# EryiXie/PlaneRecNet

Measured on AMD Instinct MI355X. Metric: img/s fwd+bwd @480×640 ResNet101-DCN, 1/2/4/8 MI355X + roofline %, higher is better.
Workload: dtype f32 (tensors and accumulation fp32; plain GEMMs and the tap-walked 4x4/s2, 1x1/s2 and sub-pixel convolutions >= 300 tiles: 2xfp16-piece split MFMA, fp32 accumulate; fp32-only rate in fp32_only_run)

## Files before the change

include/prn.h:

```cpp
#ifndef PRN_H
#define PRN_H
#include <stdint.h>
#ifdef __cplusplus
extern "C" {
#endif

#define PRN_BN_SPLITS 32

int prn_version(void);
const char* prn_last_error(void);

enum { PRN_IN_ZERO = 0, PRN_IN_REFLECT = 1, PRN_IN_UP2_REFLECT = 2, PRN_IN_DILATED = 3, PRN_IN_UP2_PHASE = 4,
       PRN_IN_EMBED1 = 5  };
enum { PRN_EPI_NONE = 0, PRN_EPI_RELU = 1, PRN_EPI_SIGMOID = 2 };

enum { PRN_SPLIT_OFF = 0, PRN_SPLIT_PLAN = 1, PRN_SPLIT_ALWAYS = 2 };
enum { PRN_PIECES_BF16 = 0, PRN_PIECES_F16 = 16 };
typedef struct prn_gemm_opts {
  int32_t split_mode;
  int32_t split_kind;
  int32_t split_products;
  int32_t split_min_tiles;
  float split_min_gflop;
  int32_t wgrad_wgs;
// ... 4 lines not shown

typedef struct prn_conv_desc {
  int32_t B, C, H, W;
  int32_t M;
  int32_t KH, KW;
  int32_t stride, pad;
  int32_t Ho, Wo;
  int32_t in_mode;
  int32_t dil;
  int32_t epilogue;
  int32_t ystride;
  int32_t yH, yW;
  int32_t reserved;
  prn_gemm_opts opts;
} prn_conv_desc;

int64_t prn_conv2d_fwd_ws_bytes(const prn_conv_desc* d);
int prn_conv2d_kernel_kind(const prn_conv_desc* d);
int prn_conv2d_fwd_partials(const prn_conv_desc* d, int64_t* offset_bytes);
int prn_gemm_pipe(int M, int K, int B, int HW, int nz, const prn_gemm_opts* opts);
int64_t prn_split_images_bytes(int M, int K, int nz);
int prn_split_prepare(const float* w, void* images, int M, int K, int nz, int kind, void* stream);
int prn_split_prepare_batched(const void* items_dev, int n_items, int64_t total_blocks, int64_t total_row_blocks, int kind, void* stream);
int prn_conv2d_fwd(const prn_conv_desc* d, const float* x, const float* w, const float* bias,
                   const float* addend, float* y, void* ws, void* stream);
#define PRN_TILE_COUNTERS 4096
int prn_conv2d_fwd_counted(const prn_conv_desc* d, const float* x, const float* w, const void* w_images, const float* bias, const float* addend, float* y,
                           void* ws, unsigned* counters, void* stream, int phase);
#define PRN_MAX_SEGMENTS 6
typedef struct prn_ragged {
  int32_t nseg;
  int32_t H[PRN_MAX_SEGMENTS], W[PRN_MAX_SEGMENTS];
} prn_ragged;
int prn_conv2d_fwd_ragged(const prn_conv_desc* d, const prn_ragged* rg, const float* x, const float* w, const float* bias,
                          const float* addend, float* y, void* stream);
int64_t prn_conv2d_wgrad_ragged_ws_bytes(const prn_conv_desc* d, const prn_ragged* rg);
int prn_conv2d_wgrad_ragged(const prn_conv_desc* d, const prn_ragged* rg, const float* x, const float* dy, float* dw, void* ws,
                            void* stream);

int prn_conv2d_fwd_phase(const prn_conv_desc* d, const float* x, const float* w, const float* bias,
                         const float* addend, float* y, void* ws, void* stream, int phase);

int prn_weight_flip_transpose(const float* w, float* wt, int M, int C, int KH, int KW, void* stream);

typedef struct prn_flip_item {
  const float* src;
// ... 274 lines not shown
```

planerecnet_amd/_lib.py:

```python
import ctypes
import os

_HERE = os.path.dirname(os.path.abspath(__file__))
LIB_PATH = os.environ.get("PRN_LIB") or os.path.join(_HERE, "libprn_hip.so")

c_int, c_float, c_void_p, c_i64 = ctypes.c_int, ctypes.c_float, ctypes.c_void_p, ctypes.c_int64


class GemmOpts(ctypes.Structure):
    _fields_ = [("split_mode", ctypes.c_int32), ("split_kind", ctypes.c_int32), ("split_products", ctypes.c_int32), ("split_min_tiles", ctypes.c_int32),
                ("split_min_gflop", ctypes.c_float), ("wgrad_wgs", ctypes.c_int32), ("wgrad_target", ctypes.c_int32), ("wgrad_split", ctypes.c_int32)]

    def key(self):
        return (self.split_mode, self.split_kind, self.split_products, self.split_min_tiles, self.split_min_gflop, self.wgrad_wgs, self.wgrad_target, self.wgrad_split)


SPLIT_OFF, SPLIT_PLAN, SPLIT_ALWAYS = 0, 1, 2
PIECES_BF16, PIECES_F16 = 0, 16


class ConvDesc(ctypes.Structure):
    _fields_ = [(n, ctypes.c_int32) for n in
                ("B", "C", "H", "W", "M", "KH", "KW", "stride", "pad", "Ho", "Wo", "in_mode", "dil", "epilogue", "ystride", "yH", "yW", "reserved")] + [
                    ("opts", GemmOpts)]
# ... 18 lines not shown
    _fields_ = [(n, ctypes.c_void_p) for n in (
        "w1", "w2", "w3", "wd", "b2", "w1_img", "w3_img", "wd_img", "u2", "u2_img", "w1_t", "w2_t", "w3_t", "wd_t", "w1_t_img", "w3_t_img", "wd_t_img", "ut2", "ut2_img",
        "w27", "b27", "w27_t", "w2_cols_t", "w2_cols_t_img")] + [(n, ctypes.c_void_p * 4) for n in ("gamma", "beta", "running_mean", "running_var")]


IN_ZERO, IN_REFLECT, IN_UP2_REFLECT, IN_DILATED, IN_UP2_PHASE, IN_EMBED1 = 0, 1, 2, 3, 4, 5
EPI_NONE, EPI_RELU, EPI_SIGMOID = 0, 1, 2
BN_SPLITS = 32

P = c_void_p
_DP = ctypes.POINTER(ConvDesc)
_OP = ctypes.POINTER(GemmOpts)
SIGNATURES = {
    "prn_version": (c_int, []),
    "prn_last_error": (ctypes.c_char_p, []),
    "prn_conv2d_fwd_ws_bytes": (c_i64, [_DP]),
    "prn_conv2d_kernel_kind": (c_int, [_DP]),
    "prn_conv2d_fwd_partials": (c_int, [_DP, ctypes.POINTER(c_i64)]),
    "prn_gemm_opts_default": (None, [_OP]),
    "prn_gemm_pipe": (c_int, [c_int, c_int, c_int, c_int, c_int, _OP]),
    "prn_split_images_bytes": (c_i64, [c_int, c_int, c_int]),
    "prn_split_prepare": (c_int, [P, P, c_int, c_int, c_int, c_int, P]),
    "prn_split_prepare_batched": (c_int, [P, c_int, c_i64, c_i64, c_int, P]),
    "prn_conv2d_fwd": (c_int, [_DP, P, P, P, P, P, P, P]),
    "prn_conv2d_fwd_ragged": (c_int, [_DP, P, P, P, P, P, P, P]),
    "prn_conv2d_wgrad_ragged_ws_bytes": (c_i64, [_DP, P]),
    "prn_conv2d_wgrad_ragged": (c_int, [_DP, P, P, P, P, P, P]),
    "prn_gn_relu_fwd_ragged": (c_int, [P, P, P, P, P, c_int, c_int, c_int, P, c_int, c_float, P]),
    "prn_gn_relu_bwd_ragged": (c_int, [P, P, P, P, P, P, P, P, c_int, c_int, c_int, P, c_int, P]),
    "prn_conv2d_fwd_phase": (c_int, [_DP, P, P, P, P, P, P, P, c_int]),
    "prn_conv2d_fwd_counted": (c_int, [_DP, P, P, P, P, P, P, P, P, P, c_int]),
    "prn_conv2d_wgrad_phase": (c_int, [_DP, P, P, P, P, P, c_int]),
    "prn_weight_flip_transpose": (c_int, [P, P, c_int, c_int, c_int, c_int, P]),
    "prn_weight_flip_transpose_batched": (c_int, [P, c_int, c_i64, P]),
    "prn_winograd_tiles": (c_i64, [c_int, c_int, c_int]),
    "prn_winograd_weights_batched": (c_int, [P, c_int, c_i64, P]),
    "prn_winograd_input": (c_int, [P, P, c_int, c_int, c_int, c_int, c_int, P]),
    "prn_gemm_batched_ws_bytes": (c_i64, [c_int, c_int, c_int, c_int, _OP]),
    "prn_gemm_batched": (c_int, [c_int, c_int, c_int, c_int, P, P, P, P, P, _OP, P]),
    "prn_winograd_output": (c_int, [P, P, P, P, c_int, c_int, c_int, c_int, c_int, P]),
    "prn_winograd_output_bn_fwd": (c_int, [P] * 8 + [c_int] * 4 + [c_float, c_float, c_int, P]),
    "prn_winograd_output_bn_bwd": (c_int, [P] * 8 + [c_int] * 5 + [P]),
    "prn_winograd_wgrad_ws_bytes": (c_i64, [c_int] * 5 + [_OP]),
    "prn_winograd_dy": (c_int, [P, P, c_int, c_int, c_int, c_int, P]),
    "prn_gemm_batched_nt_splits": (c_int, [c_int] * 4 + [_OP]),
    "prn_gemm_batched_nt_kind": (c_int, [c_int] * 4 + [_OP]),
# ... 131 lines not shown
```

planerecnet_amd/blocks.py:

```python
import ctypes
import os
import sys

import torch

from . import _lib, ops, profiling
from ._lib import lib, check

ENABLED = os.environ.get("PRN_BLOCKS", "1") == "1"
HANDOVER = os.environ.get("PRN_BLOCK_HANDOVER", "1") == "1"
SCATTER_ACCUMULATE = os.environ.get("PRN_SCATTER_ACC", "1") == "1"
STATS = {"fwd": 0, "bwd": 0, "resolved": 0, "vouched": 0, "scatter_acc": 0}

BLK_WINOGRAD, BLK_HANDOVER, BLK_KEEP_V, BLK_SCATTER_ACC = 1, 2, 4, 8
CONV2_DIRECT, CONV2_WINOGRAD, CONV2_DCN = 0, 1, 2
(I_SAVE, I_GSAVE, I_FWD_WS, I_BWD_WS, I_HO, I_WO, I_CONV2, I_KEEPS_V, I_A1, I_V, I_A2, I_OM, I_TABLE, I_D1, I_D2, I_D3, I_DD, I_DOM, I_BN_FLOATS, I_HANDOVERS,
 I_W1_IMG, I_W3_IMG, I_WD_IMG, I_W1T_IMG, I_W3T_IMG, I_WDT_IMG, I_U_IMG, I_COLT_IMG, INFO_COUNT) = range(29)

_SCRATCH = {}
_F32 = torch.float32
_empty = torch.empty


def scratch(nbytes, dev):
# ... 199 lines not shown
        save = _empty(st.save_n, device=dev, dtype=_F32)
        ws = scratch(st.fwd_ws, dev)
        rc = lib.prn_bottleneck_train_fwd(st.plan_ref, st.params_ref, x.data_ptr(), y.data_ptr(), save.data_ptr(), ws.data_ptr(), ops._raw_stream(dev.index))
        if rc:
            check(rc, "prn_bottleneck_train_fwd")
        torch._C._increment_version(st.stat_bufs)
        for m in st.bns:
            ops._count_batch(m)
        ctx.save_for_backward(x, y, save)
        ctx.st, ctx.keep, ctx.vs = st, st.keep, vs
        STATS["fwd"] += 1
        if hand_back:
            ctx.set_materialize_grads(False)
            return y, x0
        return y

    @staticmethod
    def backward(ctx, dy, dfork=None):
        x, y, save = ctx.saved_tensors
        st = ctx.st
        ps = st.ps
        if dy is None:
            return (dfork,) + (None,) * (3 + len(ps))
        if [w._version for w in st.convw] != ctx.vs:
            raise RuntimeError("a parameter of a Bottleneck block was modified between its forward and its backward pass")
        dev = x.device
        if not dy.is_contiguous():
            dy = dy.contiguous()
        info = st.info
        acc = 0
        if dfork is not None and st.hb and SCATTER_ACCUMULATE and dfork.is_contiguous() and dfork._base is None and dfork.shape == x.shape \
                and dfork.dtype == _F32 and dfork._use_count() <= _OWNED[0] and sys.getrefcount(dfork) <= _OWNED[1]:
            dx, acc, dfork = dfork, 1, None
            STATS["scatter_acc"] += 1
        else:
            dx = torch.empty_like(x)
        gsave = _empty(st.gsave_n, device=dev, dtype=_F32)
        bn_buf = _empty(st.bn_n, device=dev, dtype=_F32)
        ws = scratch(st.bwd_ws, dev)
        rc = lib.prn_bottleneck_train_bwd(st.plan_ref, st.params_ref, x.data_ptr(), y.data_ptr(), dy.data_ptr(), dx.data_ptr(), acc, save.data_ptr(), gsave.data_ptr(),
                                          bn_buf.data_ptr(), ws.data_ptr(), ops._raw_stream(dev.index))
        if rc:
            check(rc, "prn_bottleneck_train_bwd")
        ctx.keep = None
        STATS["bwd"] += 1
        if dfork is not None:
# ... 121 lines not shown
```

planerecnet_amd/csrc/prn_gemm_split.hip:

```cpp
#include "prn_common.h"
#include <stdlib.h>

namespace {

typedef __attribute__((ext_vector_type(8))) __bf16 bf16x8_t;
typedef __attribute__((ext_vector_type(16))) float f32x16_t;
typedef int i32x4_t __attribute__((ext_vector_type(4)));
typedef float f32x4_t __attribute__((ext_vector_type(4)));

constexpr int BM = 128, BK = 32;
constexpr int IMG_U4 = 1536;

__device__ __forceinline__ void split2(float x0, float x1, unsigned& h, unsigned& m, unsigned& l) {
  const unsigned u0 = __float_as_uint(x0), u1 = __float_as_uint(x1);
  const float r0 = x0 - __uint_as_float(u0 & 0xffff0000u), r1 = x1 - __uint_as_float(u1 & 0xffff0000u);
  const unsigned v0 = __float_as_uint(r0), v1 = __float_as_uint(r1);
  const float s0 = r0 - __uint_as_float(v0 & 0xffff0000u), s1 = r1 - __uint_as_float(v1 & 0xffff0000u);
  h = __builtin_amdgcn_perm(u1, u0, 0x07060302u);
  m = __builtin_amdgcn_perm(v1, v0, 0x07060302u);
  l = __builtin_amdgcn_perm(__float_as_uint(s1), __float_as_uint(s0), 0x07060302u);
}

__global__ void split_prepare_kernel(const float* __restrict__ w, uint4* __restrict__ img, int M, int K, long long zw, int mtiles, int kslices, long long total) {
  const long long i = (long long)blockIdx.x * 256 + threadIdx.x;
// ... 510 lines not shown
  const long long i = ((long long)blockIdx.x - it.first) * 256 + threadIdx.x;
  if (i >= total) return;
  const int* ex = (const int*)((const char*)it.dst + (long long)it.nz * mtiles * kslices * IMG16_U4 * 16);
  const int g = i % 4; const int r = (i / 4) % 128; const long long t = i / 512;
  const int ks = t % kslices; const long long zm = t / kslices; const int mt = zm % mtiles; const long long z = zm / mtiles;
  const int m = mt * 128 + r, k0 = ks * 32 + g * 8;
  const int sh = 14 - ex[z * (mtiles * 128) + m];
  float v[8];
  const float* wr = it.src + z * (long long)it.M * it.K + (long long)m * it.K + k0;
  if (m < it.M && k0 + 8 <= it.K && (it.K & 3) == 0 && (reinterpret_cast<uintptr_t>(it.src) & 15) == 0) {
    const float4 a = *reinterpret_cast<const float4*>(wr), b = *reinterpret_cast<const float4*>(wr + 4);
    v[0] = ldexpf(a.x, sh); v[1] = ldexpf(a.y, sh); v[2] = ldexpf(a.z, sh); v[3] = ldexpf(a.w, sh);
    v[4] = ldexpf(b.x, sh); v[5] = ldexpf(b.y, sh); v[6] = ldexpf(b.z, sh); v[7] = ldexpf(b.w, sh);
  } else {
#pragma unroll
    for (int j = 0; j < 8; ++j) v[j] = (m < it.M && k0 + j < it.K) ? ldexpf(wr[j], sh) : 0.f;
  }
  uint4 h, l;
  split2_f16(v[0], v[1], h.x, l.x); split2_f16(v[2], v[3], h.y, l.y); split2_f16(v[4], v[5], h.z, l.z); split2_f16(v[6], v[7], h.w, l.w);
  uint4* o = it.dst + t * IMG16_U4;
  o[g * 128 + r] = h; o[(4 + g) * 128 + r] = l;
}

}

int prn_split_gemm_plan(int M, int K, int B, int HW, int nz, const prn_gemm_opts* o) {
  if (o == nullptr || o->split_mode == PRN_SPLIT_OFF) return 0;
  if (M <= 0 || K <= 0 || B <= 0 || HW <= 0 || nz <= 0) return 0;
  if ((int64_t)K * HW >= (1LL << 29) || (int64_t)M * HW >= (1LL << 29)) return 0;
  const int mtiles = cdiv(M, 128), kslices = cdiv(K, 32);
  const int64_t tiles = (int64_t)mtiles * cdiv(HW, 128) * B * nz;
  int splits = 1;
  if (tiles < 300) {
    splits = (int)(640 / (tiles > 0 ? tiles : 1));
    if (splits > kslices / 8) splits = kslices / 8;
    static const int smax = prn_env_int("PRN_SPLIT_KSPLIT_MAX", 3);
    const int wide = splits > 4 ? 4 : splits;
    if (splits > smax) splits = smax;
    if (o->split_mode == PRN_SPLIT_PLAN && tiles * splits < o->split_min_tiles && tiles * wide >= o->split_min_tiles) splits = wide;
    if (splits < 1) splits = 1;
  }
  if (o->split_mode == PRN_SPLIT_ALWAYS) return splits;
  if ((int64_t)mtiles * 128 * 4 > (int64_t)M * 5) return 0;
  if (2.0 * M * K * (double)HW * B * nz < (double)o->split_min_gflop * 1e9) return 0;
  if (tiles * splits < o->split_min_tiles) return 0;
  return splits;
}
extern "C" void prn_gemm_opts_default(prn_gemm_opts* o) {
  if (!o) return;
  o->split_mode = PRN_SPLIT_PLAN; o->split_kind = PRN_PIECES_F16; o->split_products = 3; o->split_min_tiles = 300; o->split_min_gflop = 4.0f;
  o->wgrad_wgs = 0; o->wgrad_target = 0; o->wgrad_split = PRN_SPLIT_PLAN;
}
extern "C" int64_t prn_split_images_bytes(int M, int K, int nz) {
  if (M <= 0 || K <= 0 || nz <= 0) return -1;
  return prn_split_gemm_image_bytes(M, K, nz);
}
extern "C" int prn_split_prepare_batched(const void* items_dev, int n_items, int64_t total_blocks, int64_t total_row_blocks, int kind, void* stream) {
  PRN_REQUIRE(items_dev && n_items > 0 && total_blocks > 0 && total_blocks < (1LL << 31), "prn_split_prepare_batched: bad arguments");
  PRN_REQUIRE(kind == PRN_PIECES_F16 || kind == PRN_PIECES_BF16, "prn_split_prepare_batched: kind is PRN_PIECES_F16 or PRN_PIECES_BF16");
  if (kind == PRN_PIECES_F16) {
    PRN_REQUIRE(total_row_blocks > 0 && total_row_blocks < (1LL << 31), "prn_split_prepare_batched: the fp16 piece format needs the row-block count");
    hipLaunchKernelGGL(split16_rowmax_batched_kernel, dim3((unsigned)total_row_blocks), dim3(256), 0, (hipStream_t)stream, (const PrepItem*)items_dev, n_items);
    hipLaunchKernelGGL(split16_prepare_batched_kernel, dim3((unsigned)total_blocks), dim3(256), 0, (hipStream_t)stream, (const PrepItem*)items_dev, n_items);
    PRN_CHECK_LAUNCH("prn_split_prepare_batched/f16");
    return 0;
  }
  hipLaunchKernelGGL(split_prepare_batched_kernel, dim3((unsigned)total_blocks), dim3(256), 0, (hipStream_t)stream, (const PrepItem*)items_dev, n_items);
  PRN_CHECK_LAUNCH("prn_split_prepare_batched");
  return 0;
}
namespace {
int cut_weight(const float* w, void* images, int M, int K, int nz, long long zw, int kind, hipStream_t st, const char* who, int taps = 1) {
  const int mtiles = cdiv(M, 128), kslices = cdiv(K, 32);
  const long long ptotal = (long long)nz * mtiles * kslices * 512;
  if (kind == PRN_PIECES_F16) {
    int* ex = (int*)((char*)images + (int64_t)nz * mtiles * kslices * IMG16_U4 * 16);
    const long long rows = (long long)nz * mtiles * 128;
    hipLaunchKernelGGL(split16_rowmax_kernel, dim3(cdiv(rows, 4)), dim3(256), 0, st, w, ex, M, K, zw, mtiles * 128, rows);
    hipLaunchKernelGGL(split16_prepare_kernel, dim3(cdiv(ptotal, 256)), dim3(256), 0, st, w, (uint4*)images, (const int*)ex, M, K, zw, mtiles, kslices, ptotal, taps);
  } else {
    hipLaunchKernelGGL(split_prepare_kernel, dim3(cdiv(ptotal, 256)), dim3(256), 0, st, w, (uint4*)images, M, K, zw, mtiles, kslices, ptotal);
  }
  PRN_CHECK_LAUNCH(who);
  return 0;
}
}
extern "C" int prn_split_prepare(const float* w, void* images, int M, int K, int nz, int kind, void* stream) {
  PRN_REQUIRE(w && images && M > 0 && K > 0 && nz > 0 && (reinterpret_cast<uintptr_t>(images) & 15) == 0, "prn_split_prepare: bad arguments");
  PRN_REQUIRE(kind == PRN_PIECES_F16 || kind == PRN_PIECES_BF16, "prn_split_prepare: kind is PRN_PIECES_F16 or PRN_PIECES_BF16");
  return cut_weight(w, images, M, K, nz, (long long)M * K, kind, (hipStream_t)stream, "prn_split_prepare");
}
// ... 106 lines not shown
```

planerecnet_amd/ops.py:

```python
import ctypes

import os
import threading
import weakref

import torch

from . import _lib, profiling
from ._lib import ConvDesc, GemmOpts, IN_ZERO, IN_REFLECT, IN_UP2_REFLECT, IN_DILATED, IN_UP2_PHASE, IN_EMBED1, EPI_NONE, EPI_RELU, EPI_SIGMOID, lib, check


_SIDE = {}
WGRAD_ASYNC = bool(int(os.environ.get("PRN_WGRAD_ASYNC", "0")))


WGRAD_WGS_ASYNC = os.environ.get("PRN_WGRAD_WGS_ASYNC", "512")


_POLICY = {"split_mode": int(os.environ.get("PRN_SPLIT_GEMM", "1")),
           "kind": _lib.PIECES_BF16 if os.environ.get("PRN_SPLIT_KIND", "f16") == "bf16" else _lib.PIECES_F16,
           "products": int(os.environ.get("PRN_SPLIT16_PRODUCTS", "3")),
           "min_gflop": float(os.environ.get("PRN_SPLIT_MIN_GFLOP", "4.0")),
           "min_tiles": int(os.environ.get("PRN_SPLIT_MIN_TILES", os.environ.get("PRN_SPLIT_MIN_TILES_EVAL", "300"))),
           "wgrad_wgs": int(os.environ.get("PRN_WGRAD_WGS", "0") or 0),
# ... 517 lines not shown
            SPLIT_STATS["hits"] += 1
            return _p(e.images)
        if cur is None or e.dims != (M, K, nz, kind):
            _split_drop(ptr, stamp=False)
            e = None
    if e is None:
        owner = t if isinstance(t, torch.nn.Parameter) else (t._base if isinstance(t._base, torch.nn.Parameter) else None)
        if owner is None and _stamp_of(ptr) is None:
            SPLIT_STATS["uncached"] += 1
            return None
        if owner is not None and owner.data_ptr() != ptr:
            return None
        e = _SplitEntry()
        e.owner = weakref.ref(owner) if owner is not None else None
        e.tensor = None if owner is not None else t
        e.ptr, e.dims = ptr, (M, K, nz, kind)
        nb = lib.prn_split_images_bytes(M, K, nz)
        e.images = torch.empty(nb, device=t.device, dtype=torch.uint8)
        _SPLIT_IMG[ptr] = e
        _SPLIT_ITEMS[0] = None
        OPERAND_EPOCH[0] += 1
        if owner is not None:
            weakref.finalize(owner, lambda p=ptr, r=e: _split_drop(p) if _SPLIT_IMG.get(p) is r else None)
    check(lib.prn_split_prepare(ctypes.c_void_p(ptr), _p(e.images), M, K, nz, kind, _stream()), "prn_split_prepare")
    e.stamp = _split_state(e)
    SPLIT_STATS["cuts"] += 1
    if os.environ.get("PRN_SPLIT_DEBUG"):
        SPLIT_STATS.setdefault("who", {}).setdefault((M, K, nz, "param" if e.owner is not None else "derived"), []).append(SPLIT_STATS["refreshes"])
    return _p(e.images)


def split_images_ptr(t, M, K, nz, cols=None):
    r = split_images(t, M, K, nz, cols)
    return None if r is None else r.value


def split_refresh_all():
    if SPLIT_CACHE == "eval" or SPLIT_CACHE in ("0", False):
        return
    if _SPLIT_POLICY.get("mode", "eval") != "train":
        return
    dead = [p for p, e in _SPLIT_IMG.items() if _split_state(e) is None]
    for p in dead:
        _split_drop(p)
    if not _SPLIT_IMG:
        return
    kind = _POLICY["kind"]
    for e in [e for e in _SPLIT_IMG.values() if e.dims[3] != kind]:
        _split_drop(e.ptr, stamp=False)
    entries = list(_SPLIT_IMG.values())
    if not entries:
        return
    if _SPLIT_ITEMS[0] is None or _SPLIT_ITEMS[1] != [id(e) for e in entries]:
        items, blocks, rblocks = _prep_items(entries, entries[0].images.device)
        _SPLIT_ITEMS[0], _SPLIT_ITEMS[1], _SPLIT_ITEMS[2] = items, [id(e) for e in entries], (blocks, rblocks)
    check(lib.prn_split_prepare_batched(_p(_SPLIT_ITEMS[0]), len(entries), _SPLIT_ITEMS[2][0], _SPLIT_ITEMS[2][1], kind, _stream()), "prn_split_prepare_batched")
    for e in entries:
        e.stamp = _split_state(e)
    SPLIT_STATS["refreshes"] += 1


def conv_fwd_raw(x, w2d, bias, addend, M, K, stride, pad, Ho, Wo, mode=IN_ZERO, dil=1, epi=EPI_NONE, scatter2=None):
    B, C, H, W = x.shape
    if scatter2 is None:
        y = torch.empty(B, M, Ho, Wo, device=x.device, dtype=torch.float32)
        d_, ref, nbytes, _, _ = _desc(B, C, H, W, M, K, stride, pad, Ho, Wo, mode, dil, epi)
        wimg = split_images(w2d, M, C, 1, (B, Ho * Wo)) if (d_.kind >= 2 and K == 1 and stride == 1) else None
    else:
        wimg = None
        y = torch.zeros(B, M, scatter2[0], scatter2[1], device=x.device, dtype=torch.float32)
        _, ref, nbytes, _, _ = _desc(B, C, H, W, M, K, stride, pad, Ho, Wo, mode, dil, epi, 2, scatter2[0], scatter2[1])
    ws = torch.empty(nbytes // 4, device=x.device, dtype=torch.float32) if nbytes else None
    cnt = _counters(x.device) if (nbytes and FUSED_SPLIT_SUM) else None
    if profiling._enabled:
        kind = lib.prn_conv2d_kernel_kind(ref)
        direct = kind == 1
        split = kind >= 2
        nb_ = 4.0 * (x.numel() + w2d.numel() + y.numel() + (addend.numel() if addend is not None else 0))
        fl = 2.0 * M * C * K * K * B * Ho * Wo / (dil * dil)
        with profiling.span("conv3x3_direct" if direct else ("split_gemm_kernel" if split else "conv_igemm_kernel"), "hbm" if direct else "mfma",
                            nb_ if direct else (split_products() * fl if split else fl), ref=None if direct else fl, nbytes=nb_,
                            tag=None if direct else ("conv", C, H, W, M, K, stride, mode, dil, B)):
# ... 38 lines not shown

def conv_wgrad_grouped_raw(xs, dys, M, K, stride, pad, mode):
    G = len(xs)
    B, C, H, W = xs[0].shape
    Ho, Wo = dys[0].shape[2:]
    dev = xs[0].device
    _, ref, _, _, _ = _desc(B, C, H, W, M, K, stride, pad, Ho, Wo, mode)
    nbytes = lib.prn_conv2d_wgrad_grouped_ws_bytes(ref, G)
    if nbytes < 0:
        raise RuntimeError(lib.prn_last_error().decode())
    dw = torch.empty(G, M, C, K, K, device=dev, dtype=torch.float32)
    ws = _wspace(nbytes, dev)
    px = (ctypes.c_void_p * G)(*[t.data_ptr() for t in xs])
    pdy = (ctypes.c_void_p * G)(*[t.data_ptr() for t in dys])
    check(lib.prn_conv2d_wgrad_grouped(ref, G, px, pdy, _p(dw), _p(ws), _stream()), "prn_conv2d_wgrad_grouped")
    return dw


_FLIP_USED = set()


def flip_transpose(w):
    _FLIP_USED.add(w.data_ptr())
    e = _FLIPPED.get(w.data_ptr())
    if e is not None and tuple(t._version for t in e[0]) == e[1] and e[2].shape[1] == w.shape[0]:
        return e[2]
    M, C, KH, KW = w.shape
    wt = torch.empty(C, M, KH, KW, device=w.device, dtype=torch.float32)
    check(lib.prn_weight_flip_transpose(_p(w), _p(wt), M, C, KH, KW, _stream()), "prn_weight_flip_transpose")
    return wt


_FLIPPED = {}


class FlippedWeights:

    def __init__(self, weights):
        self.weights = [(e[0], tuple(int(v) for v in e[1])) for e in weights]
        self.data = [e[2] if len(e) > 2 else e[0] for e in weights]
        self.guards = [(e[0],) + tuple(e[3] if len(e) > 3 else ()) for e in weights]
        self.ptrs = None

    def _build(self):
        import numpy as np
        dev = self.weights[0][0].device
        total = sum(M * C * KH * KW for _, (M, C, KH, KW) in self.weights)
        self.flat = torch.empty(total, device=dev, dtype=torch.float32)
        items = np.zeros(len(self.weights), dtype=np.dtype([("src", "u8"), ("dst", "u8"), ("M", "i4"), ("C", "i4"), ("KH", "i4"), ("KW", "i4"),
                                                             ("first", "i8")]))
        self.views, first, blocks = [], 0, 0
        for i, ((_, (M, C, KH, KW)), w) in enumerate(zip(self.weights, self.data)):
            assert w.is_contiguous() and w.numel() == M * C * KH * KW and w.dtype == torch.float32
            v = self.flat[first:first + w.numel()].view(C, M, KH, KW)
            items[i] = (w.data_ptr(), v.data_ptr(), M, C, KH, KW, blocks)
            self.views.append(v)
            first += w.numel()
            blocks += ((M + 31) // 32) * ((C + 31) // 32)
        self.items = torch.from_numpy(items.view(np.uint8).reshape(-1).copy()).to(dev)
        self.total = blocks
        self.ptrs = [w.data_ptr() for w in self.data]
        OPERAND_EPOCH[0] += 1
        for k in [k for k, o in BATCHED.items() if o == id(self)]:
            del BATCHED[k]
        for v in self.views:
            BATCHED[v.data_ptr()] = id(self)

    def refresh(self):
        if not self.weights:
            return
        if self.ptrs is None or any(w.data_ptr() != p for w, p in zip(self.data, self.ptrs)):
            for p in (self.ptrs or []):
                _FLIPPED.pop(p, None)
            for v in (getattr(self, "views", None) or []):
                _split_drop(v.data_ptr())
            self._build()
        check(lib.prn_weight_flip_transpose_batched(_p(self.items), len(self.weights), self.total, _stream()), "prn_weight_flip_transpose_batched")
        for gd, d, v in zip(self.guards, self.data, self.views):
            _FLIPPED[d.data_ptr()] = (gd, tuple(t._version for t in gd), v)
            _stamp(v)


WINOGRAD = bool(int(os.environ.get("PRN_WINOGRAD", "1")))
WINOGRAD_WGRAD = bool(int(os.environ.get("PRN_WINOGRAD_WGRAD", "1")))
WINOGRAD_MIN_TILES = int(os.environ.get("PRN_WINOGRAD_MIN_TILES", "128"))
_WINO = {}


def winograd_ok(B, C, H, W, M, K, stride, pad, mode, epi):
    return (WINOGRAD and K == 3 and stride == 1 and pad == 1 and mode in (IN_ZERO, IN_REFLECT) and epi in (EPI_NONE, EPI_RELU)
            and W % 4 == 0 and H >= 8 and C >= 64 and M >= 64 and B * ((H + 3) // 4) * (W // 4) >= WINOGRAD_MIN_TILES)


def _winograd_items(entries, dev):
    import numpy as np
    items = np.zeros(len(entries), dtype=np.dtype([("src", "u8"), ("u", "u8"), ("ut", "u8"), ("M", "i4"), ("C", "i4"), ("first", "i8")]))
    blocks = 0
    for i, (w, M, C, U, Ut) in enumerate(entries):
        items[i] = (w.data_ptr(), U.data_ptr() if U is not None else 0, Ut.data_ptr() if Ut is not None else 0, M, C, blocks)
# ... 45 lines not shown


class WinogradWeights:

    def __init__(self, weights):
        self.weights = [w for w in weights]
        self.ptrs = None

    def _build(self):
        dev = self.weights[0].device
        total = sum(w.numel() * 4 for w in self.weights)
        self.flat_u = torch.empty(total, device=dev, dtype=torch.float32)
        self.flat_ut = torch.empty(total, device=dev, dtype=torch.float32)
        self.views, entries, first = [], [], 0
        for w in self.weights:
            M, C = w.shape[:2]
            assert w.is_contiguous() and tuple(w.shape[2:]) == (3, 3) and w.dtype == torch.float32
            n = 36 * M * C
            U, Ut = self.flat_u[first:first + n].view(36, M, C), self.flat_ut[first:first + n].view(36, C, M)
            self.views.append((U, Ut))
            entries.append((w, M, C, U, Ut))
            first += n
        self.items, self.total = _winograd_items(entries, dev)
        self.ptrs = [w.data_ptr() for w in self.weights]
        OPERAND_EPOCH[0] += 1
        for k in [k for k, o in BATCHED.items() if o == id(self)]:
            del BATCHED[k]
        for U, Ut in self.views:
            BATCHED[U.data_ptr()] = BATCHED[Ut.data_ptr()] = id(self)

    def refresh(self):
        if not self.weights or not WINOGRAD:
            return
        if self.ptrs is None or any(w.data_ptr() != p for w, p in zip(self.weights, self.ptrs)):
            for p in (self.ptrs or []):
                _wino_pop(p)
            self._build()
        check(lib.prn_winograd_weights_batched(_p(self.items), len(self.weights), self.total, _stream()), "prn_winograd_weights_batched")
        for w, (U, Ut) in zip(self.weights, self.views):
            _wino_store(w, U, Ut)


_WINO_WG_WS = {}
WINOGRAD_SPLIT_MIN_TILES = int(os.environ.get("PRN_SPLIT_WINO_MIN_TILES", "0"))
SPLIT_SKIP = set(filter(None, os.environ.get("PRN_SPLIT_SKIP", "").split(",")))
WINOGRAD_KEEP_V = int(os.environ.get("PRN_WINOGRAD_KEEP_V", str(128 << 20)))


def conv3x3_winograd_raw(x, U, bias, addend, M, mode=IN_ZERO, epi=EPI_NONE, keep=None):
    B, C, H, W = x.shape
    if mode == IN_EMBED1:
        H, W = H + 2, W + 4
    P = lib.prn_winograd_tiles(B, H, W)
    y = torch.empty(B, M, H, W, device=x.device, dtype=torch.float32)
    split_ok = "wino" not in SPLIT_SKIP and gemm_pipe(M, C, 1, P, 36) >= 1 and ((M + 127) // 128) * ((P + 127) // 128) * 36 >= WINOGRAD_SPLIT_MIN_TILES
    uimg = split_images(U, M, C, 36, (1, P)) if split_ok else None
    oref = opts_ref() if split_ok else None
    wkey = ("wino-fwd", B, C, H, W, M, opts_key() if split_ok else None)
    nb_ws = _WINO_WG_WS.get(wkey)
    if nb_ws is None:
        nb_ws = _WINO_WG_WS[wkey] = lib.prn_conv3x3_winograd_ws_bytes(B, C, H, W, M, oref)
        if nb_ws < 0:
            raise RuntimeError(lib.prn_last_error().decode())
# ... 35 lines not shown
            check(lib.prn_conv3x3_winograd_wgrad(*args, 1), "prn_conv3x3_winograd_wgrad")
        w16 = lib.prn_gemm_batched_nt_kind(M, C, P, 36, oref) == 2
        with profiling.span("wgrad16_kernel" if w16 else "conv_wgrad_kernel", "mfma", (split_products() if w16 else 1.0) * 2.0 * 36 * M * C * P, 2.0 * 9 * M * C * B * H * W,
                            tag=("wino-wgrad-products", C, H, W, M, 3, 1, mode, 1, B)):
            check(lib.prn_conv3x3_winograd_wgrad(*args, 2), "prn_conv3x3_winograd_wgrad")
        with profiling.span("winograd_dw_kernel", "hbm", float(nbytes) - 4.0 * 36 * (C + M) * P + 4.0 * dw.numel(), 0.0):
            check(lib.prn_conv3x3_winograd_wgrad(*args, 3), "prn_conv3x3_winograd_wgrad")
    else:
        check(lib.prn_conv3x3_winograd_wgrad(*args, 0), "prn_conv3x3_winograd_wgrad")
    return dw


def channel_sum(g):
    B, C, H, W = g.shape
    out = torch.empty(C, device=g.device, dtype=torch.float32)
    ws = _wspace(8 * C * _lib.BN_SPLITS, g.device, torch.float64)
    check(lib.prn_channel_sum(_p(g), _p(out), _p(ws), B, C, H * W, _stream()), "prn_channel_sum")
    return out


def conv_dgrad_raw(dy, w, x_shape, stride, pad, mode, addend=None):
    B, C, H, W = x_shape
    M, _, K, _ = w.shape
    if mode == IN_ZERO and winograd_ok(B, M, H, W, C, K, stride, pad, IN_ZERO, EPI_NONE) and tuple(dy.shape[2:]) == (H, W):
        return conv3x3_winograd_raw(dy, winograd_weights(w)[1], None, addend, C)
    wt = flip_transpose(w)
    if mode == IN_REFLECT and W % 4 == 0 and tuple(dy.shape[2:]) == (H, W) and winograd_ok(B, M, H + 2, W + 4, C, K, 1, 1, IN_ZERO, EPI_NONE):
        dp = conv3x3_winograd_raw(dy, winograd_weights(w)[1], None, None, C, IN_EMBED1)
        dx = torch.empty(B, C, H, W, device=dy.device, dtype=torch.float32)
        check(lib.prn_pad_fold_pitched(_p(dp), _p(dx), B, C, H, W, W + 4, _stream()), "prn_pad_fold_pitched")
        return dx if addend is None else dx + addend
    if mode in (IN_REFLECT, IN_UP2_REFLECT):
        Hv, Wv = (2 * H, 2 * W) if mode == IN_UP2_REFLECT else (H, W)
        dp = conv_fwd_raw(dy, wt, None, None, C, K, 1, 2, Hv + 2, Wv + 2)
        dx = torch.empty(B, C, H, W, device=dy.device, dtype=torch.float32)
        check(lib.prn_pad_fold(_p(dp), _p(dx), B, C, H, W, 1 if mode == IN_UP2_REFLECT else 0, _stream()), "prn_pad_fold")
        return dx if addend is None else dx + addend
    if stride == 1:
        return conv_fwd_raw(dy, wt, None, addend, C, K, 1, K - 1 - pad, H, W)
    if stride != 2:
        raise RuntimeError("conv dgrad: stride %d not implemented" % stride)
    if K == 1 and pad == 0 and addend is None:
        return conv_fwd_raw(dy, wt, None, None, C, 1, 1, 0, dy.shape[2], dy.shape[3], scatter2=(H, W))
    if K == 1 and pad == 0:
        return conv_fwd_raw(dy, wt, None, None, C, 1, 1, 0, dy.shape[2], dy.shape[3], scatter2=(H, W)) + addend
    return conv_fwd_raw(dy, wt, None, addend, C, K, 1, K - 1 - pad, H, W, IN_DILATED, 2)
# ... 684 lines not shown
class _RaggedConv(torch.autograd.Function):
    @staticmethod
    def forward(ctx, xp, w, bias, rs):
        _dev(xp, w, bias)
        xp, w, bias = _c(xp), _c(w), _c(bias)
        M, C, K, _ = w.shape
        assert xp.numel() == rs.pixels * C, (xp.shape, w.shape, rs.sizes)
        P = rs.winograd(C, M, K)
        y = _ragged_winograd_raw(xp, winograd_weights(w)[0], bias, None, rs, C, M, P) if P else _ragged_conv_raw(xp, w, bias, None, rs, C, M, K)
        ctx.save_for_backward(xp, w)
        ctx.rs, ctx.has_bias = rs, bias is not None
        ctx.bias = bias
        return y

    @staticmethod
    def backward(ctx, dy):
        xp, w = ctx.saved_tensors
        rs = ctx.rs
        dy = _c(dy)
        M, C, K, _ = w.shape
        dx = dw = db = None
        P = rs.winograd(C, M, K)
        if ctx.needs_input_grad[0]:
            dx = _ragged_winograd_raw(dy, winograd_weights(w)[1], None, None, rs, M, C, P) if P else _ragged_conv_raw(dy, flip_transpose(w), None, None, rs, M, C, K)
        def wgrad():
            if P and WINOGRAD_WGRAD:
                oref = opts_ref()
                key = (rs.key, C, M, opts_key())
                nb = _WINO_WG_WS.get(key)
                if nb is None:
                    nb = _WINO_WG_WS[key] = lib.prn_winograd_wgrad_ragged_ws_bytes(rs.ref, rs.B, C, M, oref)
                ws = torch.empty(nb // 4, device=xp.device, dtype=torch.float32)
                dwo = torch.empty_like(w)
                with profiling.span("conv3x3_winograd_wgrad_ragged", "mfma", 2.0 * 36 * M * C * P, 2.0 * 9 * M * C * rs.pixels):
                    check(lib.prn_conv3x3_winograd_wgrad_ragged(_p(xp), _p(dy), _p(dwo), _p(ws), rs.ref, rs.B, C, M, oref, _stream()), "prn_conv3x3_winograd_wgrad_ragged")
                return dwo
            _, ref, nbytes = _rdesc(rs, C, M, K)
            ws = torch.empty(max(nbytes // 4, 1), device=xp.device, dtype=torch.float32)
            dwo = torch.empty_like(w)
            with profiling.span("conv_wgrad_kernel", "mfma", 2.0 * M * C * K * K * rs.pixels):
                check(lib.prn_conv2d_wgrad_ragged(ref, rs.ref, _p(xp), _p(dy), _p(dwo), _p(ws), _stream()), "prn_conv2d_wgrad_ragged")
            return dwo
        if _defer(ctx.needs_input_grad[1], w):
            _deferred_wgrad(w, (xp, dy), wgrad)
        elif ctx.needs_input_grad[1]:
            dw = wgrad()
# ... 129 lines not shown
```

planerecnet_amd/planerecnet.py:

```python
import os

import torch
import torch.nn as nn
import torch.nn.functional as F

from . import ops, timer
from .backbone import can_fold, construct_backbone, conv_bn, folded_bn
from .config import cfg
from .fpn import FPN
from .funcs import bias_init_with_prob
from .nms import mask_nms, matrix_nms


_COORD = {}


def _coord_channels(feat):
    B, _, h, w = feat.shape
    key = (B, h, w, feat.device)
    c = _COORD.get(key)
    if c is None:
        xr = torch.linspace(-1, 1, w, device=feat.device)
        yr = torch.linspace(-1, 1, h, device=feat.device)
        y, x = torch.meshgrid(yr, xr, indexing="ij")
# ... 51 lines not shown
            dcns = [m for m in self.modules() if isinstance(m, DeformableConv2d)]
            dcn_w = {id(m.regular_conv.weight) for m in dcns}
            dcn_om = {id(c.weight) for m in dcns for c in (m.offset_conv, m.modulator_conv)}
            items = []
            for m in self.modules():
                if isinstance(m, nn.Conv2d) and m.weight.requires_grad and m.weight.is_cuda and id(m.weight) not in dcn_om:
                    M, C, KH, KW = m.weight.shape
                    items.append((m.weight, (M, C * KH * KW, 1, 1) if id(m.weight) in dcn_w else (M, C, KH, KW)))
            for m in dcns:
                if m.offset_conv.weight.requires_grad and m.offset_conv.weight.is_cuda:
                    w27 = m._merged()[0]
                    items.append((m.offset_conv.weight, tuple(w27.shape), w27, (m.modulator_conv.weight,)))
            self.__dict__["_flip_dcn"] = [(m, e[2]) for m, e in zip([m for m in dcns if m.offset_conv.weight.requires_grad and m.offset_conv.weight.is_cuda],
                                                                     [e for e in items if len(e) > 2])]
            fw = self.__dict__["_flipped"] = ops.FlippedWeights(items)
            self.__dict__["_flip_steps"] = 0
        self.__dict__["_flip_steps"] += 1
        if self.__dict__["_flip_steps"] == 3:
            used = [(w, shp, d, gd[1:]) for (w, shp), d, gd in zip(fw.weights, fw.data, fw.guards) if d.data_ptr() in ops._FLIP_USED]
            if used and len(used) < len(fw.weights):
                for d in fw.data:
                    ops._FLIPPED.pop(d.data_ptr(), None)
                fw = self.__dict__["_flipped"] = ops.FlippedWeights(used)
        fw.refresh()
        mine = self.__dict__.get("_param_ids")
        if mine is None:
            mine = self.__dict__["_param_ids"] = {id(p) for p in self.parameters()}
        seen = [w for w in ops.winograd_seen() if id(w) in mine]
        ww = self.__dict__.get("_wino")
        if seen and (ww is None or len(ww.weights) != len(seen)):
            ww = self.__dict__["_wino"] = ops.WinogradWeights(seen)
        if ww is not None:
            ww.refresh()
        ops.split_refresh_all()
        ops.vouch_refreshed([t for gd in fw.guards for t in gd])
        if ww is not None:
            ops.vouch_refreshed(ww.weights)

    def forward(self, x):
        if x.is_cuda:
            ops.split_gemm_policy("train" if self.training else "eval")
        if self.training and torch.is_grad_enabled() and x.is_cuda:
            self._refresh_dgrad_weights()
        with timer.env("backbone"):
            enc = self.backbone(x)
        with timer.env("fpn"):
            feats, fenc = self.fpn([enc[i] for i in self.fpn_indices], return_inputs=True)
            enc = list(enc)
            for i, f in zip(self.fpn_indices, fenc):
                enc[i] = f
        with timer.env("instance head"):
            ins_feats, feats[0] = self.split_feats([feats[f] for f in range(len(self.instance_in_features))], fork=True)
            cate_pred, kernel_pred = self.inst_head(ins_feats)
        with timer.env("mask head"):
            mask_pred = self.mask_head([feats[f] for f in range(len(self.mask_in_features))])
        with timer.env("depth_decoder"):
            depth_pred = self.depth_decoder([enc[i] for i in self.depth_decoder_indices], mask_pred, kernel_pred)
        with timer.env("Inferencing"):
            if self.training:
                return mask_pred, cate_pred, kernel_pred, depth_pred
            from .metrics import category_scores
            return self.inference(mask_pred, category_scores(cate_pred), kernel_pred, depth_pred, x)

    @staticmethod
    def split_feats(feats, fork=False):
        h, w = feats[0].shape[2:]
        if fork:
            r, f0 = ops.resize_bilinear_fork(feats[0], (int(h * 0.5), int(w * 0.5)))
            return (r, feats[1], feats[2], feats[3]), f0
        return (ops.resize_bilinear(feats[0], (int(h * 0.5), int(w * 0.5))), feats[1], feats[2], feats[3])

    def _flush_bn_counters(self):
        for m in self.modules():
            if isinstance(m, nn.BatchNorm2d):
                ops.flush_batch_count(m)

    def state_dict(self, *args, **kwargs):
        self._flush_bn_counters()
        return super().state_dict(*args, **kwargs)

    def load_state_dict(self, *args, **kwargs):
        for m in self.modules():
# ... 349 lines not shown
```

Measured before the change: 194.6.

## Refresh backward-only derived weights on a side stream and fuse split-image prep

```diff
diff --git a/include/prn.h b/include/prn.h
--- a/include/prn.h
+++ b/include/prn.h
@@ -50,6 +50,13 @@
 int64_t prn_split_images_bytes(int M, int K, int nz);
 int prn_split_prepare(const float* w, void* images, int M, int K, int nz, int kind, void* stream);
 int prn_split_prepare_batched(const void* items_dev, int n_items, int64_t total_blocks, int64_t total_row_blocks, int kind, void* stream);
+typedef struct prn_refresh_item {
+  const float* src;
+  void* images;
+  int32_t M, K, nz, pad;
+  int64_t first;
+} prn_refresh_item;
+int prn_weight_refresh_batched(const prn_refresh_item* items_host, const void* items_dev, int n_items, int kind, void* stream);
 int prn_conv2d_fwd(const prn_conv_desc* d, const float* x, const float* w, const float* bias,
                    const float* addend, float* y, void* ws, void* stream);
 #define PRN_TILE_COUNTERS 4096
diff --git a/planerecnet_amd/_lib.py b/planerecnet_amd/_lib.py
--- a/planerecnet_amd/_lib.py
+++ b/planerecnet_amd/_lib.py
@@ -64,6 +64,7 @@
     "prn_split_images_bytes": (c_i64, [c_int, c_int, c_int]),
     "prn_split_prepare": (c_int, [P, P, c_int, c_int, c_int, c_int, P]),
     "prn_split_prepare_batched": (c_int, [P, c_int, c_i64, c_i64, c_int, P]),
+    "prn_weight_refresh_batched": (c_int, [P, P, c_int, c_int, P]),
     "prn_conv2d_fwd": (c_int, [_DP, P, P, P, P, P, P, P]),
     "prn_conv2d_fwd_ragged": (c_int, [_DP, P, P, P, P, P, P, P]),
     "prn_conv2d_wgrad_ragged_ws_bytes": (c_i64, [_DP, P]),
diff --git a/planerecnet_amd/blocks.py b/planerecnet_amd/blocks.py
--- a/planerecnet_amd/blocks.py
+++ b/planerecnet_amd/blocks.py
@@ -245,6 +245,7 @@
         ps = st.ps
         if dy is None:
             return (dfork,) + (None,) * (3 + len(ps))
+        ops.backward_join()
         if [w._version for w in st.convw] != ctx.vs:
             raise RuntimeError("a parameter of a Bottleneck block was modified between its forward and its backward pass")
         dev = x.device
diff --git a/planerecnet_amd/csrc/prn_gemm_split.hip b/planerecnet_amd/csrc/prn_gemm_split.hip
--- a/planerecnet_amd/csrc/prn_gemm_split.hip
+++ b/planerecnet_amd/csrc/prn_gemm_split.hip
@@ -556,6 +556,87 @@
   o[g * 128 + r] = h; o[(4 + g) * 128 + r] = l;
 }
 
+constexpr int RF_HELD = 4;
+__device__ __forceinline__ void refresh_load8(const float* wr, bool vec, bool row_ok, int k0, int K, float* v) {
+  if (row_ok && vec && k0 + 8 <= K) {
+    const float4 a = *reinterpret_cast<const float4*>(wr + k0), b = *reinterpret_cast<const float4*>(wr + k0 + 4);
+    v[0] = a.x; v[1] = a.y; v[2] = a.z; v[3] = a.w; v[4] = b.x; v[5] = b.y; v[6] = b.z; v[7] = b.w;
+  } else {
+#pragma unroll
+    for (int j = 0; j < 8; ++j) v[j] = (row_ok && k0 + j < K) ? wr[k0 + j] : 0.f;
+  }
+}
+template <int KIND>
+__global__ __launch_bounds__(256) void weight_refresh_kernel(const prn_refresh_item* __restrict__ items, int n) {
+  __shared__ float rowmx[4][16];
+  int lo = 0, hi = n - 1;
+  const long long blk = blockIdx.x;
+  while (lo < hi) { const int mid = (lo + hi + 1) >> 1; if (items[mid].first <= blk) lo = mid; else hi = mid - 1; }
+  const prn_refresh_item it = items[lo];
+  const int mtiles = (it.M + 127) / 128, kslices = (it.K + 31) / 32, Mpad = mtiles * 128;
+  const long long u = blk - it.first;
+  const int rg = (int)(u % 8); const long long zm = u / 8; const int mt = (int)(zm % mtiles); const long long z = zm / mtiles;
+  if (z >= it.nz) return;
+  const int lane = threadIdx.x & 63, wave = threadIdx.x >> 6;
+  const int g = lane & 3, r = rg * 16 + (lane >> 2), m = mt * 128 + r;
+  const bool row_ok = m < it.M;
+  const bool vec = (it.K & 3) == 0 && (reinterpret_cast<uintptr_t>(it.src) & 15) == 0;
+  const float* wr = it.src + z * (long long)it.M * it.K + (long long)(row_ok ? m : 0) * it.K;
+  float held[RF_HELD][8];
+#pragma unroll
+  for (int i = 0; i < RF_HELD; ++i) {
+    const int ks = wave + 4 * i;
+    refresh_load8(wr, vec, row_ok && ks < kslices, ks * 32 + g * 8, it.K, held[i]);
+  }
+  int sh = 0;
+  if (KIND == PRN_PIECES_F16) {
+    float mx = 0.f;
+#pragma unroll
+    for (int i = 0; i < RF_HELD; ++i)
+#pragma unroll
+      for (int j = 0; j < 8; ++j) mx = fmaxf(mx, fabsf(held[i][j]));
+    for (int ks = wave + 4 * RF_HELD; ks < kslices; ks += 4) {
+      float v[8];
+      refresh_load8(wr, vec, row_ok, ks * 32 + g * 8, it.K, v);
+#pragma unroll
+      for (int j = 0; j < 8; ++j) mx = fmaxf(mx, fabsf(v[j]));
+    }
+    mx = fmaxf(mx, __shfl_xor(mx, 1, 64)); mx = fmaxf(mx, __shfl_xor(mx, 2, 64));
+    if (g == 0) rowmx[wave][lane >> 2] = mx;
+    __syncthreads();
+    const int rr = lane >> 2;
+    mx = fmaxf(fmaxf(rowmx[0][rr], rowmx[1][rr]), fmaxf(rowmx[2][rr], rowmx[3][rr]));
+    const int e = mx > 0.f ? __builtin_amdgcn_frexp_expf(mx) : 0;
+    int* ex = (int*)((char*)it.images + (long long)it.nz * mtiles * kslices * IMG16_U4 * 16);
+    if (wave == 0 && g == 0) ex[z * Mpad + m] = e;
+    sh = 14 - e;
+  }
+  const long long t0 = (z * mtiles + mt) * kslices;
+  auto emit = [&](int ks, float* v) {
+    if (KIND == PRN_PIECES_F16) {
+#pragma unroll
+      for (int j = 0; j < 8; ++j) v[j] = (row_ok && ks * 32 + g * 8 + j < it.K) ? ldexpf(v[j], sh) : 0.f;
+      uint4 h, l;
+      split2_f16(v[0], v[1], h.x, l.x); split2_f16(v[2], v[3], h.y, l.y); split2_f16(v[4], v[5], h.z, l.z); split2_f16(v[6], v[7], h.w, l.w);
+      uint4* o = (uint4*)it.images + (t0 + ks) * IMG16_U4;
+      o[g * 128 + r] = h; o[(4 + g) * 128 + r] = l;
+    } else {
+      uint4 h, mm, l;
+      split2(v[0], v[1], h.x, mm.x, l.x); split2(v[2], v[3], h.y, mm.y, l.y); split2(v[4], v[5], h.z, mm.z, l.z); split2(v[6], v[7], h.w, mm.w, l.w);
+      uint4* o = (uint4*)it.images + (t0 + ks) * IMG_U4;
+      o[(0 * 4 + g) * 128 + r] = h; o[(1 * 4 + g) * 128 + r] = mm; o[(2 * 4 + g) * 128 + r] = l;
+    }
+  };
+#pragma unroll
+  for (int i = 0; i < RF_HELD; ++i)
+    if (wave + 4 * i < kslices) emit(wave + 4 * i, held[i]);
+  for (int ks = wave + 4 * RF_HELD; ks < kslices; ks += 4) {
+    float v[8];
+    refresh_load8(wr, vec, row_ok, ks * 32 + g * 8, it.K, v);
+    emit(ks, v);
+  }
+}
+
 }
 
 int prn_split_gemm_plan(int M, int K, int B, int HW, int nz, const prn_gemm_opts* o) {
@@ -601,6 +682,26 @@
   }
   hipLaunchKernelGGL(split_prepare_batched_kernel, dim3((unsigned)total_blocks), dim3(256), 0, (hipStream_t)stream, (const PrepItem*)items_dev, n_items);
   PRN_CHECK_LAUNCH("prn_split_prepare_batched");
+  return 0;
+}
+extern "C" int prn_weight_refresh_batched(const prn_refresh_item* items_host, const void* items_dev, int n_items, int kind, void* stream) {
+  PRN_REQUIRE(items_host && items_dev && n_items > 0, "prn_weight_refresh_batched: null table or no items");
+  PRN_REQUIRE(kind == PRN_PIECES_F16 || kind == PRN_PIECES_BF16, "prn_weight_refresh_batched: kind is PRN_PIECES_F16 or PRN_PIECES_BF16");
+  int64_t blocks = 0;
+  for (int i = 0; i < n_items; ++i) {
+    const prn_refresh_item& it = items_host[i];
+    PRN_REQUIRE(it.src && it.images, "prn_weight_refresh_batched: item %d: null source or images", i);
+    PRN_REQUIRE((reinterpret_cast<uintptr_t>(it.images) & 15) == 0 && (reinterpret_cast<uintptr_t>(it.src) & 3) == 0, "prn_weight_refresh_batched: item %d: images are not 16-byte aligned", i);
+    PRN_REQUIRE(it.M > 0 && it.K > 0 && it.nz > 0, "prn_weight_refresh_batched: item %d: M, K, nz must be positive", i);
+    PRN_REQUIRE(it.first == blocks, "prn_weight_refresh_batched: item %d: `first` is not the running workgroup count", i);
+    blocks += (int64_t)it.nz * cdiv(it.M, 128) * 8;
+    PRN_REQUIRE(blocks < (1LL << 31), "prn_weight_refresh_batched: too many workgroups");
+  }
+  if (kind == PRN_PIECES_F16)
+    hipLaunchKernelGGL(weight_refresh_kernel<PRN_PIECES_F16>, dim3((unsigned)blocks), dim3(256), 0, (hipStream_t)stream, (const prn_refresh_item*)items_dev, n_items);
+  else
+    hipLaunchKernelGGL(weight_refresh_kernel<PRN_PIECES_BF16>, dim3((unsigned)blocks), dim3(256), 0, (hipStream_t)stream, (const prn_refresh_item*)items_dev, n_items);
+  PRN_CHECK_LAUNCH("prn_weight_refresh_batched");
   return 0;
 }
 namespace {
diff --git a/planerecnet_amd/ops.py b/planerecnet_amd/ops.py
--- a/planerecnet_amd/ops.py
+++ b/planerecnet_amd/ops.py
@@ -563,6 +563,8 @@
         OPERAND_EPOCH[0] += 1
         if owner is not None:
             weakref.finalize(owner, lambda p=ptr, r=e: _split_drop(p) if _SPLIT_IMG.get(p) is r else None)
+    if ptr in _BWD_OPERANDS:
+        backward_join()
     check(lib.prn_split_prepare(ctypes.c_void_p(ptr), _p(e.images), M, K, nz, kind, _stream()), "prn_split_prepare")
     e.stamp = _split_state(e)
     SPLIT_STATS["cuts"] += 1
@@ -576,7 +578,24 @@
     return None if r is None else r.value
 
 
-def split_refresh_all():
+REFRESH_FUSED = bool(int(os.environ.get("PRN_REFRESH_FUSED", "1")))
+_BWD_OPERANDS = set()
+_BWD_EVENT = [None, set()]
+_REFRESH_ITEMS = {}
+
+
+def _refresh_items(entries, dev):
+    import numpy as np
+    items = np.zeros(len(entries), dtype=np.dtype([("src", "u8"), ("images", "u8"), ("M", "i4"), ("K", "i4"), ("nz", "i4"), ("pad", "i4"), ("first", "i8")]))
+    blocks = 0
+    for i, e in enumerate(entries):
+        M, K, nz, _ = e.dims
+        items[i] = (e.ptr, e.images.data_ptr(), M, K, nz, 0, blocks)
+        blocks += nz * ((M + 127) // 128) * 8
+    return items, torch.from_numpy(items.view(np.uint8).reshape(-1).copy()).to(dev)
+
+
+def split_refresh_all(part=None):
     if SPLIT_CACHE == "eval" or SPLIT_CACHE in ("0", False):
         return
     if _SPLIT_POLICY.get("mode", "eval") != "train":
@@ -590,15 +609,59 @@
     for e in [e for e in _SPLIT_IMG.values() if e.dims[3] != kind]:
         _split_drop(e.ptr, stamp=False)
     entries = list(_SPLIT_IMG.values())
+    if part is not None:
+        entries = [e for e in entries if (e.ptr in _BWD_OPERANDS) == (part == "bwd")]
     if not entries:
         return
-    if _SPLIT_ITEMS[0] is None or _SPLIT_ITEMS[1] != [id(e) for e in entries]:
-        items, blocks, rblocks = _prep_items(entries, entries[0].images.device)
-        _SPLIT_ITEMS[0], _SPLIT_ITEMS[1], _SPLIT_ITEMS[2] = items, [id(e) for e in entries], (blocks, rblocks)
-    check(lib.prn_split_prepare_batched(_p(_SPLIT_ITEMS[0]), len(entries), _SPLIT_ITEMS[2][0], _SPLIT_ITEMS[2][1], kind, _stream()), "prn_split_prepare_batched")
+    ids = [id(e) for e in entries]
+    if REFRESH_FUSED:
+        tab = _REFRESH_ITEMS.get(part)
+        if tab is None or tab[0] != ids:
+            tab = _REFRESH_ITEMS[part] = (ids,) + _refresh_items(entries, entries[0].images.device)
+        check(lib.prn_weight_refresh_batched(ctypes.c_void_p(tab[1].ctypes.data), _p(tab[2]), len(entries), kind, _stream()), "prn_weight_refresh_batched")
+    else:
+        if _SPLIT_ITEMS[0] is None or _SPLIT_ITEMS[1] != ids:
+            items, blocks, rblocks = _prep_items(entries, entries[0].images.device)
+            _SPLIT_ITEMS[0], _SPLIT_ITEMS[1], _SPLIT_ITEMS[2] = items, ids, (blocks, rblocks)
+        check(lib.prn_split_prepare_batched(_p(_SPLIT_ITEMS[0]), len(entries), _SPLIT_ITEMS[2][0], _SPLIT_ITEMS[2][1], kind, _stream()), "prn_split_prepare_batched")
     for e in entries:
         e.stamp = _split_state(e)
     SPLIT_STATS["refreshes"] += 1
+
+
+def refresh_derived(fw, ww, side_ok):
+    if not (REFRESH_FUSED and side_ok):
+        fw.refresh()
+        if ww is not None:
+            ww.refresh()
+        split_refresh_all()
+        return
+    fw.ensure()
+    if ww is not None:
+        ww.ensure()
+        ww.refresh("u")
+    split_refresh_all("fwd")
+    main = torch.cuda.current_stream()
+    side = _side_stream(main.device, main)
+    side.wait_stream(main)
+    with torch.cuda.stream(side):
+        fw.refresh()
+        if ww is not None:
+            ww.refresh("ut")
+        split_refresh_all("bwd")
+        ev = torch.cuda.Event()
+        ev.record(side)
+    _BWD_EVENT[0], _BWD_EVENT[1] = ev, set()
+
+
+def backward_join():
+    ev = _BWD_EVENT[0]
+    if ev is None:
+        return
+    st = torch.cuda.current_stream()
+    if st.cuda_stream not in _BWD_EVENT[1]:
+        st.wait_event(ev)
+        _BWD_EVENT[1].add(st.cuda_stream)
 
 
 def conv_fwd_raw(x, w2d, bias, addend, M, K, stride, pad, Ho, Wo, mode=IN_ZERO, dil=1, epi=EPI_NONE, scatter2=None):
@@ -683,6 +746,7 @@
 
 def flip_transpose(w):
     _FLIP_USED.add(w.data_ptr())
+    backward_join()
     e = _FLIPPED.get(w.data_ptr())
     if e is not None and tuple(t._version for t in e[0]) == e[1] and e[2].shape[1] == w.shape[0]:
         return e[2]
@@ -726,16 +790,21 @@
             del BATCHED[k]
         for v in self.views:
             BATCHED[v.data_ptr()] = id(self)
-
-    def refresh(self):
-        if not self.weights:
-            return
-        if self.ptrs is None or any(w.data_ptr() != p for w, p in zip(self.data, self.ptrs)):
+            _BWD_OPERANDS.add(v.data_ptr())
+
+    def ensure(self):
+        if self.weights and (self.ptrs is None or any(w.data_ptr() != p for w, p in zip(self.data, self.ptrs))):
             for p in (self.ptrs or []):
                 _FLIPPED.pop(p, None)
             for v in (getattr(self, "views", None) or []):
                 _split_drop(v.data_ptr())
+                _BWD_OPERANDS.discard(v.data_ptr())
             self._build()
+
+    def refresh(self):
+        if not self.weights:
+            return
+        self.ensure()
         check(lib.prn_weight_flip_transpose_batched(_p(self.items), len(self.weights), self.total, _stream()), "prn_weight_flip_transpose_batched")
         for gd, d, v in zip(self.guards, self.data, self.views):
             _FLIPPED[d.data_ptr()] = (gd, tuple(t._version for t in gd), v)
@@ -827,23 +896,42 @@
             entries.append((w, M, C, U, Ut))
             first += n
         self.items, self.total = _winograd_items(entries, dev)
+        self.items_part = {"u": _winograd_items([(w, M, C, U, None) for w, M, C, U, _ in entries], dev)[0],
+                           "ut": _winograd_items([(w, M, C, None, Ut) for w, M, C, _, Ut in entries], dev)[0]}
         self.ptrs = [w.data_ptr() for w in self.weights]
         OPERAND_EPOCH[0] += 1
         for k in [k for k, o in BATCHED.items() if o == id(self)]:
             del BATCHED[k]
         for U, Ut in self.views:
             BATCHED[U.data_ptr()] = BATCHED[Ut.data_ptr()] = id(self)
-
-    def refresh(self):
+            _BWD_OPERANDS.add(Ut.data_ptr())
+
+    def ensure(self):
+        if self.weights and WINOGRAD and (self.ptrs is None or any(w.data_ptr() != p for w, p in zip(self.weights, self.ptrs))):
+            for p in (self.ptrs or []):
+                _wino_pop(p)
+            for _, Ut in (getattr(self, "views", None) or []):
+                _BWD_OPERANDS.discard(Ut.data_ptr())
+            self._build()
+
+    def refresh(self, part=None):
         if not self.weights or not WINOGRAD:
             return
-        if self.ptrs is None or any(w.data_ptr() != p for w, p in zip(self.weights, self.ptrs)):
-            for p in (self.ptrs or []):
-                _wino_pop(p)
-            self._build()
-        check(lib.prn_winograd_weights_batched(_p(self.items), len(self.weights), self.total, _stream()), "prn_winograd_weights_batched")
+        self.ensure()
+        items = self.items if part is None else self.items_part[part]
+        check(lib.prn_winograd_weights_batched(_p(items), len(self.weights), self.total, _stream()), "prn_winograd_weights_batched")
         for w, (U, Ut) in zip(self.weights, self.views):
-            _wino_store(w, U, Ut)
+            if part == "u":
+                _stamp(U)
+            elif part == "ut":
+                _stamp(Ut)
+                e = _WINO.get(w.data_ptr())
+                if e is not None and e[0]() is w and e[2] is U and e[3] is Ut:
+                    _WINO[w.data_ptr()] = (e[0], w._version, U, Ut)
+                else:
+                    _wino_store(w, U, Ut)
+            else:
+                _wino_store(w, U, Ut)
 
 
 _WINO_WG_WS = {}
@@ -925,6 +1013,7 @@
 def conv_dgrad_raw(dy, w, x_shape, stride, pad, mode, addend=None):
     B, C, H, W = x_shape
     M, _, K, _ = w.shape
+    backward_join()
     if mode == IN_ZERO and winograd_ok(B, M, H, W, C, K, stride, pad, IN_ZERO, EPI_NONE) and tuple(dy.shape[2:]) == (H, W):
         return conv3x3_winograd_raw(dy, winograd_weights(w)[1], None, addend, C)
     wt = flip_transpose(w)
@@ -1655,6 +1744,7 @@
         dx = dw = db = None
         P = rs.winograd(C, M, K)
         if ctx.needs_input_grad[0]:
+            backward_join()
             dx = _ragged_winograd_raw(dy, winograd_weights(w)[1], None, None, rs, M, C, P) if P else _ragged_conv_raw(dy, flip_transpose(w), None, None, rs, M, C, K)
         def wgrad():
             if P and WINOGRAD_WGRAD:
diff --git a/planerecnet_amd/planerecnet.py b/planerecnet_amd/planerecnet.py
--- a/planerecnet_amd/planerecnet.py
+++ b/planerecnet_amd/planerecnet.py
@@ -97,7 +97,6 @@
                 for d in fw.data:
                     ops._FLIPPED.pop(d.data_ptr(), None)
                 fw = self.__dict__["_flipped"] = ops.FlippedWeights(used)
-        fw.refresh()
         mine = self.__dict__.get("_param_ids")
         if mine is None:
             mine = self.__dict__["_param_ids"] = {id(p) for p in self.parameters()}
@@ -105,9 +104,7 @@
         ww = self.__dict__.get("_wino")
         if seen and (ww is None or len(ww.weights) != len(seen)):
             ww = self.__dict__["_wino"] = ops.WinogradWeights(seen)
-        if ww is not None:
-            ww.refresh()
-        ops.split_refresh_all()
+        ops.refresh_derived(fw, ww, self.__dict__["_flip_steps"] > 3)
         ops.vouch_refreshed([t for gd in fw.guards for t in gd])
         if ww is not None:
             ops.vouch_refreshed(ww.weights)
@@ -133,6 +130,8 @@
             depth_pred = self.depth_decoder([enc[i] for i in self.depth_decoder_indices], mask_pred, kernel_pred)
         with timer.env("Inferencing"):
             if self.training:
+                if x.is_cuda:
+                    ops.backward_join()
                 return mask_pred, cate_pred, kernel_pred, depth_pred
             from .metrics import category_scores
             return self.inference(mask_pred, category_scores(cate_pred), kernel_pred, depth_pred, x)
```

Result: no change. 194.6, median of 4 (+0.0%).
